# pvjosue/CWFA

Measured on AMD Instinct MI355X. Metric: volumes/sec inverse-pass @512×512×96 fp32; NLL match vs ref (1/2/4/8 GPU), higher is better.
Workload: dtype f32 (storage, accumulation, wavelets, couplings); convolution products on the bf16 matrix cores from an exact three-way bf16 split of both fp32 operands, six products per fp32 product: fp32-equivalent; plain-fp32-MFMA figure: fp32_mfma; 1 GPU; 512x512x96 volume, 4-scale CWFA (CAT blocks, 64 ch) + LRNN inverse, z=0, batch 1/GPU, random-init weights (BASELINE.json configs[2]); precision=split, parallelism=replicated x1 (independent volumes per GPU, no collective)

## Files before the change

cwfa_amd/build.py:

```python
import os
import subprocess
import sys
from concurrent.futures import ThreadPoolExecutor

HERE = os.path.dirname(os.path.abspath(__file__))
CSRC = os.path.join(HERE, "csrc")
INCLUDE = os.path.join(os.path.dirname(HERE), "include")
LIB = os.path.join(HERE, "libcwfa_hip.so")
SOURCES = ["elementwise.hip", "conv2d.hip", "conv_wino.hip", "conv_wino2d.hip", "conv_split_layer.hip", "conv_split_out.hip", "conv_split3x3.hip", "conv3d.hip", "conv3d_split.hip", "lrnn_ops.hip", "conv_bwd.hip", "eval_ops.hip", "prep_ops.hip", "optim_ops.hip", "loss_ops.hip", "deconv_ops.hip", "neuron_ops.hip", "noise_ops.hip"]
HIPCC = os.environ.get("HIPCC", "/opt/rocm/bin/hipcc")
FLAGS = ["--offload-arch=gfx950", "-O3", "-fPIC", "-std=c++17", "-ffp-contract=off", "-I", INCLUDE, "-I", CSRC,
         "-Wall", "-Wno-unused-function"]


EXTRA = {"conv3d_split.hip": ["-fno-slp-vectorize"]}


def _newer(src, dst):
    return not os.path.exists(dst) or os.path.getmtime(src) > os.path.getmtime(dst)


def build_all(force=False, verbose=False):
    deps = [os.path.join(CSRC, "common.h"), os.path.join(CSRC, "conv_internal.h"), os.path.join(CSRC, "conv_split_out_geom.h"), os.path.join(INCLUDE, "cwfa_hip.h"),
            os.path.abspath(__file__)]
    objs, jobs = [], []
    for s in SOURCES:
        src, obj = os.path.join(CSRC, s), os.path.join(CSRC, s.replace(".hip", ".o"))
        objs.append(obj)
        if force or _newer(src, obj) or any(_newer(d, obj) for d in deps):
            jobs.append([HIPCC, *FLAGS, *EXTRA.get(s, []), "-c", src, "-o", obj])

    def run(cmd):
        if verbose:
            print(" ".join(cmd), flush=True)
        r = subprocess.run(cmd, capture_output=True, text=True)
        if r.returncode != 0:
            raise RuntimeError(f"hipcc failed: {' '.join(cmd)}\n{r.stdout}\n{r.stderr}")
        return r.stderr
# ... 13 lines not shown
```

cwfa_amd/csrc/conv2d.hip:

```cpp
#include "conv_internal.h"

#include <string.h>
#include <type_traits>

namespace {

template <int KS_, int CK_, int MT_, int NT_, int WM_, int WN_, int XV_ = 1>
struct Cfg {
    static constexpr int KS = KS_, CK = CK_, MT = MT_, NT = NT_, WM = WM_, WN = WN_;
    static constexpr int XV = XV_;
    static_assert(XV_ == 1 || (XV_ == 4 && KS_ == 1), "vector staging needs halo-free tiles");
    static constexpr int PAD = KS / 2;
    static constexpr int NTHREADS = 64 * WM * WN;
    static constexpr int CT = 32 * MT * WM;
    static constexpr int TR = NT * WN;
    static constexpr int TC = 32;
    static constexpr int XR = TR + KS - 1;
    static constexpr int XC = TC + KS - 1;
    static constexpr int XS = CK * XR * XC;
    static constexpr int XS_PAD = (XS + 3) & ~3;
    static constexpr int WS = KS * KS * CK * CT;
    static constexpr int XPT = (XS / XV + NTHREADS - 1) / NTHREADS;
    static constexpr int WPT = (WS / 4 + NTHREADS - 1) / NTHREADS;
    static constexpr int BUF = XS_PAD + WS;
// ... 541 lines not shown
            return CWFA_E_SHAPE;
        default: break;
    }
    return launch_epi<C, EPI_GENERIC, PRO>(p, st);
}

template <class C, unsigned ALLOWED, unsigned ALLOWED_PRO>
int launch(const ConvParams& p, int epi, hipStream_t st) {
    if (p.o.in_scale || p.o.in_add) return launch_sel<C, ALLOWED_PRO, true>(p, epi, st);
    return launch_sel<C, ALLOWED, false>(p, epi, st);
}

}
int g_cwfa_split_xcd_map = 1;
int g_cwfa_split_rows16 = 1;
extern int g_cwfa_mip3_ablate;
namespace {

int fill_params(ConvParams& p, const char* name, const float* x, const float* w_packed, float* y, int B, int Cin, int H,
                int W, int Cout, int64_t x_bs, int64_t y_bs, const cwfa_conv_opts* opts) {
    CWFA_REQUIRE(B >= 0 && Cin > 0 && Cout > 0 && H >= 0 && W >= 0, CWFA_E_INVAL, "%s: bad size", name);
    if (B == 0 || H == 0 || W == 0) return 1;
    CWFA_REQUIRE(x && w_packed && y, CWFA_E_INVAL, "%s: null pointer", name);
    CWFA_REQUIRE(!opts || !opts->out_sample_stats, CWFA_E_INVAL, "%s: out_sample_stats is a feature of the few-channel cwfa_conv7x7_split_f32", name);
    CWFA_REQUIRE((int64_t)Cin * H * W < (1ll << 30) && (int64_t)Cout * H * W * (p.o.upshuffle2 ? 1 : 1) < (1ll << 30), CWFA_E_SHAPE, "%s: C*H*W exceeds the 32-bit byte offsets of a tile (2^30 elements per image)", name);
    CWFA_REQUIRE(cwfa_aligned16(w_packed), CWFA_E_ALIGN, "%s: packed weights must be 16-byte aligned", name);
    p.x = x; p.wp = w_packed; p.y = y;
    p.B = B; p.Cin = Cin; p.H = H; p.W = W; p.Cout = Cout;
    p.x_bs = x_bs; p.y_bs = y_bs;
    p.products = g_cwfa_operand == CwfaOperand::split3 ? 6 : 1;
// ... 308 lines not shown
    }
    if (strcmp(name, "winograd_2d") == 0) {
        g_cwfa_wino_2d = value;
        return CWFA_OK;
    }
    if (strcmp(name, "wgrad_split") == 0) {
        g_cwfa_wgrad_split = value != 0;
        return CWFA_OK;
    }
    if (strcmp(name, "wgrad_rows") == 0) {
        g_cwfa_wgrad_rows = value;
        return CWFA_OK;
    }
    if (strcmp(name, "split3x3_xcd_map") == 0) {
        g_cwfa_split_xcd_map = value;
        return CWFA_OK;
    }
    if (strcmp(name, "mip3_ablate") == 0) {
        CWFA_REQUIRE(value >= 0 && value <= 7, CWFA_E_INVAL, "cwfa_set_option: mip3_ablate is a mask of bits 0..2");
        g_cwfa_mip3_ablate = value;
        return CWFA_OK;
    }
    if (strcmp(name, "split3x3_rows16") == 0) {
        g_cwfa_split_rows16 = value;
        return CWFA_OK;
    }
    if (strcmp(name, "split_products") == 0) {
        CWFA_REQUIRE(value == 1 || value == 6, CWFA_E_INVAL, "cwfa_set_option: split_products must be 1 or 6");
        CWFA_REQUIRE(value == 1 || g_cwfa_operand != CwfaOperand::fp16, CWFA_E_INVAL,
                     "cwfa_set_option: split_products = 6 needs split_operand = 0 (the three-piece split is a bf16 format)");
// ... 130 lines not shown
```

cwfa_amd/csrc/conv_split3x3.hip:

```cpp
#include "conv_internal.h"

extern int g_cwfa_split_xcd_map;
extern int g_cwfa_split_rows16;

namespace {

constexpr int TR = 8, TC = 32;

template <int KS, int RPW = 4>
struct XG {
    static constexpr int TRW = 2 * RPW, NT = 2 * RPW;
    static constexpr int PAD = KS / 2, XR = TRW + 2 * PAD, XC = TC + 2 * PAD, NTAP = KS * KS;
    static constexpr int EPK = XR * XC;
    static constexpr int KHB = KS == 7 ? 8512 : RPW == 8 ? 9792 : 5440;
    static constexpr int XPB = 2 * KHB;
    static constexpr int XB = 3 * XPB;
    static constexpr bool SPECIAL = KS == 3 && RPW == 4;
    static constexpr int NEK = SPECIAL ? 2 : 3;
    static_assert(EPK * 16 <= KHB && KHB % 256 == 64 && 2 * EPK <= 512 * NEK, "staging entry map");
    static_assert(!SPECIAL || (EPK > 256 && EPK <= 384), "3x3 staging entry map");
    static_assert(KS == 3 || RPW == 4, "7x7: 8-row tiles");
};

template <int MPW, int KS = 3, int RPW = 4, int WM = 4>
struct Geo {
    static constexpr int CT = 16 * MPW * WM;
    static constexpr int WSL = 3 * 4 * CT * 16;
    static constexpr int LDS = 2 * XG<KS, RPW>::XB + 2 * WSL;
    static_assert(LDS <= 160 * 1024, "LDS budget");
};

struct SParams {
    const float* x;
    const void* wp;
    float* y;
    int B, Cin, H, W, Cout, nchunks, nsteps, tiles_x, ntiles, ctiles, xcd_map;
    int nrun;
    int64_t x_bs, y_bs;
    cwfa_conv_opts o;
    cwfa_couple cp;
};

template <int KS, int RPW>
__host__ __device__ constexpr int tap_off(int buf, int tap) { return buf * XG<KS, RPW>::XB + ((tap / KS) * XG<KS, RPW>::XC + tap % KS) * 16; }

enum { EPI_RUNTIME = -1, EPI_COUPLE = -2 };

template <int MPW, bool SIX, bool ADD, int ACT1, int KS = 3, int RPW = 4, int WM = 4, bool F16 = false>
__global__ __launch_bounds__(512, 1) void conv3x3_split_kernel(SParams p) {
    typedef XG<KS, RPW> G;
    constexpr int XC = G::XC, EPK = G::EPK, KHB = G::KHB, XPB = G::XPB, XB = G::XB, NTAP = G::NTAP, PAD = G::PAD;
    constexpr int WN = 8 / WM, RW = G::TRW / WN, NT = 2 * RW;
    constexpr bool SPECIAL = G::SPECIAL;
    static_assert(SPECIAL || ((MPW == 1 || WM != 4) && !ADD), "7x7 / 16-row tiles: the 64-channel and narrow tilings, without a skip add");
    static_assert(WM == 4 || (((KS == 3 && RPW == 8) || KS == 7) && MPW <= 3 && !ADD && ACT1 != EPI_COUPLE),
                  "narrow tilings: 16-row tile (7x7: 8-row), <= 3 m-tiles per wave");
    static_assert(MPW != 3 || WM != 4, "three m-tiles per wave: the 48- / 96-channel tilings only");
    constexpr int CT = 16 * MPW * WM;
    constexpr int WSL = 3 * 4 * CT * 16;
    extern __shared__ __attribute__((aligned(16))) char lds[];
    const int tid = threadIdx.x, lane = tid & 63, c16 = lane & 15, g = lane >> 4;
    const int wave = __builtin_amdgcn_readfirstlane(tid >> 6);
    const int wm = wave % WM, wn = wave / WM;
    const int HW = p.H * p.W;
    const int plane = HW * 4;
    constexpr unsigned OOB = 0x80000000u;
    constexpr int NQ = SIX ? 3 : 1;
    constexpr int OFF_W = 2 * XB;
    const int b = blockIdx.z;
    int sp, ct;
    if (p.xcd_map && (p.ntiles & 7) == 0) {
        const int xcd = blockIdx.x & 7, slot = blockIdx.x >> 3;
        sp = xcd * (p.ntiles >> 3) + slot / p.ctiles;
        ct = slot % p.ctiles;
    } else {
        sp = blockIdx.x / p.ctiles;
        ct = blockIdx.x % p.ctiles;
    }
    const int row0 = (sp / p.tiles_x) * G::TRW, col0 = (sp % p.tiles_x) * TC;

    constexpr int NEK = G::NEK;
    int ekh[NEK], eidx[NEK];
    bool fin[NEK];
    unsigned fo[NEK];
    if constexpr (SPECIAL) {
        ekh[0] = wave >> 2; eidx[0] = tid & 255; fin[0] = true;
        ekh[1] = (wave >> 1) & 1; eidx[1] = 256 + (tid & 127); fin[1] = wave < 4 && eidx[1] < EPK;
    } else {
#pragma unroll
        for (int k = 0; k < NEK; ++k) {
            const int e = tid + 512 * k;
            ekh[k] = e >= EPK;
            eidx[k] = e - ekh[k] * EPK;
            fin[k] = e < 2 * EPK;
        }
    }
    bool fok[NEK];
#pragma unroll
    for (int k = 0; k < NEK; ++k) {
        const int r = eidx[k] / XC, c = eidx[k] % XC;
        const int gr = row0 + r - PAD, gc = col0 + c - PAD;
        fok[k] = fin[k] && gr >= 0 && gr < p.H && gc >= 0 && gc < p.W;
        fo[k] = !fok[k] ? OOB : p.o.in_blocked8 ? (unsigned)((gr * p.W + gc) * 32) : (unsigned)((gr * p.W + gc) * 4);
        if constexpr (!SPECIAL) fo[k] = !fok[k] ? OOB : fo[k] + (unsigned)(ekh[k] * 8) * (unsigned)plane;
    }
    const int xbytes = p.Cin * plane;
    const auto rx = CWFA_RSRC(p.x + (int64_t)b * p.x_bs, xbytes);
    const auto ra = CWFA_RSRC(ADD ? p.o.in_add + (int64_t)b * p.o.in_add_bs : p.x, ADD ? xbytes : 0);
    const bool has_aff = p.o.in_scale != nullptr;
    typedef const float __attribute__((address_space(4))) cfloat;
    cfloat* sc = has_aff ? (cfloat*)(p.o.in_scale + (int64_t)b * p.o.in_affine_bs) : nullptr;
    cfloat* sh = has_aff ? (cfloat*)(p.o.in_shift + (int64_t)b * p.o.in_affine_bs) : nullptr;

    auto load_entry = [&](auto kc, float (&xv)[8], float (&av)[8], int chunk) {
        constexpr int k = decltype(kc)::value;
        const int ch0 = chunk * 16 + (SPECIAL ? ekh[k] * 8 : 0);
        if (KS == 3 && !ADD && p.o.in_blocked8) {
            const f32x4 lo4 = __builtin_bit_cast(f32x4, __builtin_amdgcn_raw_buffer_load_b128(rx, fo[k], ch0 * plane, 0));
            const f32x4 hi4 = __builtin_bit_cast(f32x4, __builtin_amdgcn_raw_buffer_load_b128(rx, fo[k], ch0 * plane + 16, 0));
#pragma unroll
            for (int j = 0; j < 4; ++j) {
                xv[j] = lo4[j];
                xv[4 + j] = hi4[j];
            }
            return;
        }
#pragma unroll
// ... 22 lines not shown
            float v = xv[j];
            if (has_aff) v = fok[k] ? v * scv[j] + shv[j] : 0.f;
            if constexpr (ADD) v += av[j];
            __bf16 a1, a2 = (__bf16)0.f, a3 = (__bf16)0.f;
            cwfa_split3<SIX, F16>(v, a1, a2, a3);
            pc[0][j] = a1; pc[1][j] = a2; pc[2][j] = a3;
        }
        char* dst = lds + buf * XB + ekh[k] * KHB + eidx[k] * 16;
        if (SPECIAL || fin[k]) {
#pragma unroll
            for (int q = 0; q < NQ; ++q) *reinterpret_cast<bf16x8*>(dst + q * XPB) = pc[q];
        }
    };

    constexpr int NPC = (SIX ? WSL : WSL / 3) / 1024;
    const int64_t wtile = (int64_t)ct * p.nsteps * WSL;
    const char* wbase = reinterpret_cast<const char*>(p.wp) + wtile;
    const auto rw = CWFA_RSRC(wbase, p.nsteps * WSL);
    auto dma_w = [&](int slice, int slot) {
        cwfa_static_for<(NPC + 7) / 8>([&](auto ic_) {
            constexpr int i = decltype(ic_)::value;
            const int piece = i * 8 + wave;
            if (piece < NPC) {
                char* dst = lds + OFF_W + slot * WSL + piece * 1024;
                __builtin_amdgcn_raw_ptr_buffer_load_lds(rw, (lds_ptr)dst, 16, (unsigned)(lane * 16), slice * WSL + piece * 1024, 0, 0);
            }
        });
    };

    const int alane = OFF_W + (g * CT + wm * MPW * 16 + c16) * 16;
    const int blane = (g & 1) * KHB + (wn * RW * XC + c16) * 16;
    const bool sel = (g >> 1) != 0;

    f32x4 acc[MPW][NT];
#pragma unroll
    for (int mt = 0; mt < MPW; ++mt)
#pragma unroll
        for (int nt = 0; nt < NT; ++nt) acc[mt][nt] = f32x4{0.f, 0.f, 0.f, 0.f};
    constexpr int NB = MPW == 4 ? 3 : 2, MA = MPW == 4 ? 2 : MPW;
    static_assert(NB - 1 < NT, "B look-ahead");
    bf16x8 A[MPW][3], Bq[NB][3];
    float xs[NEK][8], sk[NEK][8];

    auto read_a = [&](int abase, int m0, int m1) {
#pragma unroll
        for (int mt = m0; mt < m1; ++mt)
#pragma unroll
            for (int q = 0; q < NQ; ++q) A[mt][q] = *reinterpret_cast<const bf16x8*>(lds + abase + (q * 4 * CT + mt * 16) * 16);
    };
    auto read_b = [&](int set, int bbase, int nt) {
#pragma unroll
        for (int q = 0; q < NQ; ++q)
            Bq[set][q] = *reinterpret_cast<const bf16x8*>(lds + bbase + q * XPB + ((nt >> 1) * XC + 16 * (nt & 1)) * 16);
    };
    auto mfma6 = [&](f32x4& c, const bf16x8 (&a)[3], const bf16x8 (&bb)[3]) {
        if constexpr (SIX) {
            CWFA_MFMA(a[2], bb[0], c);
            CWFA_MFMA(a[1], bb[1], c);
            CWFA_MFMA(a[0], bb[2], c);
            CWFA_MFMA(a[1], bb[0], c);
            CWFA_MFMA(a[0], bb[1], c);
        }
        CWFA_MFMA_OP(F16, a[0], bb[0], c);
    };

    {
        float x0[NEK][8], s0[NEK][8];
        cwfa_static_for<NEK>([&](auto kc) { load_entry(kc, x0[decltype(kc)::value], s0[decltype(kc)::value], 0); });
        cwfa_static_for<NEK>([&](auto kc) { load_entry(kc, xs[decltype(kc)::value], sk[decltype(kc)::value], 1); });
        dma_w(0, 0);
        cwfa_static_for<NEK>([&](auto kc) { store_entry(kc, x0[decltype(kc)::value], s0[decltype(kc)::value], 0, 0); });
    }
    asm volatile("s_waitcnt vmcnt(0)\n\ts_waitcnt lgkmcnt(0)" ::: "memory");
    __builtin_amdgcn_s_barrier();

    read_b(0, blane + (sel ? tap_off<KS, RPW>(0, 1) : tap_off<KS, RPW>(0, 0)), 0);
    int sl = 0, P = 0, ce = 0;
    for (int step = 0; step < p.nrun; ++step) {
        const int co = ce + 1;
        const int uA = 2 * P, uB = 2 * P + 1;
        const int bufA = uA >= NTAP, tA = uA - NTAP * bufA, bufB = uB >= NTAP, tB = uB - NTAP * bufB;
        const int offA = bufA * XB + ((tA / KS) * XC + tA % KS) * 16, offB = bufB * XB + ((tB / KS) * XC + tB % KS) * 16;
        constexpr int SB = 0, SA = KS == 3 ? 5 : 26, LA = KS == 3 ? 2 : 22, LB = KS == 3 ? 6 : 44;
        static_assert(LB + NEK - 1 < NTAP && LA + NEK - 1 < SA, "staging schedule");
        static_assert(SB < LA && SA <= LB, "staging schedule: one register set per entry (a step's stores come before its loads)");
        {
            const bool odd0 = P == SB, odd1 = P == SB + 1;
            if (odd0 || P == SA) store_entry(cwfa_ic<0>{}, xs[0], sk[0], odd0 ? co : ce + 2, odd0);
            if (odd1 || P == SA + 1) store_entry(cwfa_ic<1>{}, xs[1], sk[1], odd1 ? co : ce + 2, odd1);
            if constexpr (NEK > 2) {
                const bool odd2 = P == SB + 2;
                if (odd2 || P == SA + 2) store_entry(cwfa_ic<NEK - 1>{}, xs[NEK - 1], sk[NEK - 1], odd2 ? co : ce + 2, odd2);
            }
        }
        CWFA_FENCE();
        const int abase = alane + sl * WSL;
        const int bbase = blane + (sel ? offB : offA);
        read_a(abase, 0, MA);
        CWFA_FENCE();
#pragma unroll
        for (int nt = 0; nt < NT; ++nt) {
            if ((MA == MPW || nt > 0) && nt + NB - 1 < NT) read_b((nt + NB - 1) % NB, bbase, nt + NB - 1);
            CWFA_FENCE();
#pragma unroll
            for (int mt = 0; mt < MPW; ++mt) {
                mfma6(acc[mt][nt], A[mt], Bq[nt % NB]);
                CWFA_FENCE();
                if (MA < MPW && nt == 0 && mt == 0) {
                    read_a(abase, MA, MPW);
#pragma unroll
                    for (int n2 = 1; n2 < NB && n2 < NT; ++n2) read_b(n2, bbase, n2);
                    CWFA_FENCE();
                }
            }
            if (nt == 0) {
                if (P == LA || P == LB) load_entry(cwfa_ic<0>{}, xs[0], sk[0], P == LA ? ce + 2 : co + 2);
                if (P == LA + 1 || P == LB + 1) load_entry(cwfa_ic<1>{}, xs[1], sk[1], P == LA + 1 ? ce + 2 : co + 2);
                if constexpr (NEK > 2) {
                    if (P == LA + 2 || P == LB + 2) load_entry(cwfa_ic<NEK - 1>{}, xs[NEK - 1], sk[NEK - 1], P == LA + 2 ? ce + 2 : co + 2);
                }
                CWFA_FENCE();
            }
            if (nt == 1) {
                dma_w(step + 1, sl ^ 1);
                CWFA_FENCE();
            }
        }
        {
            const int nP = P == NTAP - 1 ? 0 : P + 1;
            const int nA = 2 * nP, nB = 2 * nP + 1;
            const int nbufA = nA >= NTAP, ntA = nA - NTAP * nbufA, nbufB = nB >= NTAP, ntB = nB - NTAP * nbufB;
            const int noffA = nbufA * XB + ((ntA / KS) * XC + ntA % KS) * 16, noffB = nbufB * XB + ((ntB / KS) * XC + ntB % KS) * 16;
            read_b(0, blane + (sel ? noffB : noffA), 0);
            CWFA_FENCE();
        }
        asm volatile("s_waitcnt vmcnt(0)" ::: "memory");
        if constexpr (SIX) asm volatile("s_waitcnt lgkmcnt(3)" ::: "memory");
        else asm volatile("s_waitcnt lgkmcnt(1)" ::: "memory");
        __builtin_amdgcn_s_barrier();
        sl ^= 1;
        if (++P == NTAP) {
            P = 0;
            ce += 2;
        }
    }
    asm volatile("s_waitcnt vmcnt(0)" ::: "memory");

    const auto ry = CWFA_RSRC(p.y + (int64_t)b * p.y_bs, p.Cout * plane);
    const auto rr = CWFA_RSRC(p.o.residual ? p.o.residual + (int64_t)b * p.o.res_bs : p.y, p.o.residual ? p.Cout * plane : 0);
    const auto rb = CWFA_RSRC(p.o.bias ? p.o.bias : p.y, p.o.bias ? p.Cout * 4 : 0);
    const bool alpha_pc = p.o.prelu_per_channel != 0;
    const float alpha = (p.o.prelu_alpha && !alpha_pc) ? *p.o.prelu_alpha : 0.f;
    const auto rpa = CWFA_RSRC(alpha_pc ? p.o.prelu_alpha : p.y, alpha_pc ? p.Cout * 4 : 0);
    const int cwave = ct * CT + wm * MPW * 16;
    const unsigned glane = (unsigned)(4 * g) * (unsigned)plane;
    if constexpr (ACT1 == EPI_COUPLE) {
        static_assert(MPW <= 2 && !ADD, "coupling epilogue: narrow tilings only");
        constexpr int NP = MPW == 1 ? 2 : 4;
        const cwfa_couple& cp = p.cp;
        const auto cx = CWFA_RSRC(cp.x + (int64_t)b * cp.x_bs, cp.n * plane);
        const auto cy = CWFA_RSRC(cp.y + (int64_t)b * cp.y_bs, cp.n * plane);
        const unsigned jlane = (unsigned)((MPW == 1 ? 2 : 4) * g) * (unsigned)plane;
        const int jwave = wm * (MPW == 1 ? 8 : 16);
        float bs[NP], bt[NP];
#pragma unroll
        for (int k = 0; k < NP; ++k) {
            const int rs = k, rt = MPW == 1 ? k + 2 : 16 + k;
            bs[k] = __builtin_bit_cast(float, __builtin_amdgcn_raw_buffer_load_b32(rb, (unsigned)(16 * g), (cwave + rs) * 4, 0));
            bt[k] = __builtin_bit_cast(float, __builtin_amdgcn_raw_buffer_load_b32(rb, (unsigned)(16 * g), (cwave + rt) * 4, 0));
        }
        float ssum = 0.f;
#pragma unroll
        for (int nt = 0; nt < NT; ++nt) {
            const int row = row0 + wn * RW + (nt >> 1), col = col0 + 16 * (nt & 1) + c16;
            const bool ok = row < p.H && col < p.W;
            const unsigned po = ok ? (unsigned)((row * p.W + col) * 4) + jlane : OOB;
            float xv[NP];
#pragma unroll
            for (int k = 0; k < NP; ++k) xv[k] = __builtin_bit_cast(float, __builtin_amdgcn_raw_buffer_load_b32(cx, po, (jwave + k) * plane, 0));
#pragma unroll
            for (int k = 0; k < NP; ++k) {
                const float sr = acc[0][nt][k] + bs[k];
                float tr;
                if constexpr (MPW == 1) tr = acc[0][nt][k + 2] + bt[k];
                else tr = acc[MPW - 1][nt][k] + bt[k];
                const float sv = cwfa_soft_clamp(sr * cp.pre_scale, cp.clamp_kind, cp.clamp);
                const float tv = tr * cp.pre_scale;
                const float yv = cp.rev ? (xv[k] - tv) * __expf(-sv) : __expf(sv) * xv[k] + tv;
                __builtin_amdgcn_raw_buffer_store_b32(__builtin_bit_cast(unsigned, yv), cy, po, (jwave + k) * plane, 0);
                ssum += ok ? sv : 0.f;
            }
            CWFA_FENCE();
        }
        if (cp.logdet) {
            const double ws = cwfa_wave_sum((double)ssum);
            double* red = reinterpret_cast<double*>(lds);
            __builtin_amdgcn_s_barrier();
            if (lane == 0) red[wave] = ws;
            __syncthreads();
            if (tid == 0) {
                double tot = 0.0;
#pragma unroll
                for (int w = 0; w < 8; ++w) tot += red[w];
                atomicAdd(&cp.logdet[b], cp.rev ? -tot : tot);
            }
        }
        return;
    }
    const bool outb = p.o.out_blocked8 != 0;
    const bool want_stats = ACT1 != EPI_RUNTIME && p.o.out_stats != nullptr;
    float* red = reinterpret_cast<float*>(lds);
#pragma unroll
    for (int mt = 0; mt < MPW; ++mt) {
        float bias[4];
        float st1[4] = {0.f, 0.f, 0.f, 0.f}, st2[4] = {0.f, 0.f, 0.f, 0.f};
#pragma unroll
        for (int r = 0; r < 4; ++r)
            bias[r] = __builtin_bit_cast(float, __builtin_amdgcn_raw_buffer_load_b32(rb, (unsigned)(16 * g), (cwave + mt * 16 + r) * 4, 0));
        float al[4] = {alpha, alpha, alpha, alpha};
        if (alpha_pc) {
#pragma unroll
            for (int r = 0; r < 4; ++r)
                al[r] = __builtin_bit_cast(float, __builtin_amdgcn_raw_buffer_load_b32(rpa, (unsigned)(16 * g), (cwave + mt * 16 + r) * 4, 0));
        }
        constexpr int RLA = NT < 4 ? NT : 4;
        float rv[ACT1 == EPI_RUNTIME ? NT : 1][4];
        auto load_res = [&](int nt) {
            const int row = row0 + wn * RW + (nt >> 1), col = col0 + 16 * (nt & 1) + c16;
            const unsigned po = (row < p.H && col < p.W) ? (unsigned)((row * p.W + col) * 4) + glane : OOB;
#pragma unroll
            for (int r = 0; r < 4; ++r)
                rv[ACT1 == EPI_RUNTIME ? nt : 0][r] = __builtin_bit_cast(float, __builtin_amdgcn_raw_buffer_load_b32(rr, po, (cwave + mt * 16 + r) * plane, 0));
        };
        if constexpr (ACT1 == EPI_RUNTIME) {
#pragma unroll
            for (int nt = 0; nt < NT; ++nt)
#pragma unroll
                for (int r = 0; r < 4; ++r) rv[nt][r] = 0.f;
            if (p.o.residual) {
#pragma unroll
                for (int nt = 0; nt < RLA; ++nt) load_res(nt);
            }
            CWFA_FENCE();
        }
#pragma unroll
        for (int nt = 0; nt < NT; ++nt) {
            const int row = row0 + wn * RW + (nt >> 1), col = col0 + 16 * (nt & 1) + c16;
            if constexpr (ACT1 == EPI_RUNTIME) {
                if (nt + RLA < NT && p.o.residual) load_res(nt + RLA);
                CWFA_FENCE();
            }
            if constexpr (ACT1 != EPI_RUNTIME) {
                if (outb) {
                    f32x4 o4;
#pragma unroll
                    for (int r = 0; r < 4; ++r) o4[r] = cwfa_act_ct<ACT1>(acc[mt][nt][r] + bias[r], al[r]);
                    const unsigned pb = (row < p.H && col < p.W) ? (unsigned)(((g >> 1) * HW + row * p.W + col) * 32 + (g & 1) * 16) : OOB;
                    cwfa_buffer_store_b128(__builtin_bit_cast(u32x4, o4), ry, pb, (cwave + mt * 16) * plane);
                    continue;
                }
            }
            const unsigned po = (row < p.H && col < p.W) ? (unsigned)((row * p.W + col) * 4) + glane : OOB;
#pragma unroll
            for (int r = 0; r < 4; ++r) {
                const int soff = (cwave + mt * 16 + r) * plane;
                float v = acc[mt][nt][r] + bias[r];
                if constexpr (ACT1 == EPI_RUNTIME) {
                    v = cwfa_act(v, p.o.act, al[r]);
                    v += rv[nt][r];
                    v = cwfa_act(v, p.o.act2, al[r]);
                } else {
                    v = cwfa_act_ct<ACT1>(v, al[r]);
                    if (want_stats) {
                        const float vm = po != OOB ? v : 0.f;
                        st1[r] += vm;
                        st2[r] += vm * vm;
                    }
                }
                __builtin_amdgcn_raw_buffer_store_b32(__builtin_bit_cast(unsigned, v), ry, po, soff, 0);
            }
            CWFA_FENCE();
        }
        if constexpr (ACT1 != EPI_RUNTIME) {
            if (want_stats) {
#pragma unroll
                for (int r = 0; r < 4; ++r) {
                    const float a1 = cwfa_row16_sum(st1[r]), a2 = cwfa_row16_sum(st2[r]);
                    if (c16 == 0) {
                        const int ch = (wm * MPW + mt) * 16 + 4 * g + r;
                        red[(wn * CT + ch) * 2] = a1;
                        red[(wn * CT + ch) * 2 + 1] = a2;
                    }
                }
            }
        }
    }
    if constexpr (ACT1 != EPI_RUNTIME) {
        if (want_stats) {
            asm volatile("s_waitcnt lgkmcnt(0)\n\ts_barrier" ::: "memory");
            const int ch = ct * CT + tid;
            if (tid < CT && ch < p.Cout) {
                double s1 = 0.0, s2 = 0.0;
#pragma unroll
                for (int k = 0; k < WN; ++k) {
                    s1 += (double)red[(k * CT + tid) * 2];
                    s2 += (double)red[(k * CT + tid) * 2 + 1];
                }
                atomicAdd(&p.o.out_stats[2 * ch], s1);
                atomicAdd(&p.o.out_stats[2 * ch + 1], s2);
            }
        }
    }
}

namespace few {
constexpr int XR = TR + 6, XC = TC + 6, EPK = XR * XC;
constexpr int XPB = EPK * 16;
constexpr int NSTEP = 13, CT = 64, MPW = 2, WM = 2, WN = 4, RW = 2, NT = 4;
constexpr int WSL = 3 * 4 * CT * 16;
constexpr int OFF_W = 3 * XPB, LDS = OFF_W + 2 * WSL;
static_assert(2 * 512 >= EPK && 2 * LDS <= 160 * 1024, "few-channel 7x7: staging map / two blocks per CU");
}

template <bool SIX, bool F16>
__global__ __launch_bounds__(512, 2) void conv7x7_few_split_kernel(SParams p) {
    using namespace few;
// ... 234 lines not shown
    for (int q = 0; q < 3; ++q) {
        uint4 v4;
        v4.x = pc[q][0] | ((unsigned)pc[q][1] << 16);
        v4.y = pc[q][2] | ((unsigned)pc[q][3] << 16);
        v4.z = pc[q][4] | ((unsigned)pc[q][5] << 16);
        v4.w = pc[q][6] | ((unsigned)pc[q][7] << 16);
        out[(((int64_t)ctile * nsteps + s) * 3 + q) * 4 * CT + g * CT + col] = v4;
    }
}

inline int mpw_of(int Cout) { return Cout > 128 ? 4 : Cout > 96 ? 2 : Cout > 64 ? 3 : Cout > 48 ? 1 : Cout > 32 ? 3 : Cout > 16 ? 2 : 1; }
inline int wm_of(int Cout) { return Cout > 96 ? 4 : Cout > 64 ? 2 : Cout > 48 ? 4 : 1; }
inline int ct_of(int Cout) { return 16 * mpw_of(Cout) * wm_of(Cout); }
inline int nsteps_of(int Cin, int ntap = 9) { return ntap * (((Cin + 15) / 16 + 1) / 2); }

template <int MPW, bool ADD, int ACT1, int KS = 3, int RPW = 4, int WM = 4>
int launch(const SParams& p, hipStream_t stream) {
    typedef Geo<MPW, KS, RPW, WM> G;
    constexpr int TRW = XG<KS, RPW>::TRW;
    const int tiles_y = (p.H + TRW - 1) / TRW, ctiles = (p.Cout + G::CT - 1) / G::CT;
    SParams q = p;
    q.ntiles = p.tiles_x * tiles_y;
    q.ctiles = ctiles;
    q.xcd_map = g_cwfa_split_xcd_map;
    if ((int64_t)q.ntiles * ctiles >= (1ll << 31)) {
        cwfa_set_error("cwfa_conv3x3_split_f32: grid too large");
        return CWFA_E_SHAPE;
    }
    if ((ACT1 == EPI_RUNTIME || ACT1 == EPI_COUPLE) && (p.o.out_stats || p.o.out_blocked8)) {
        cwfa_set_error("cwfa_conv3x3_split_f32: out_stats / out_blocked8 reached a run-time epilogue");
        return CWFA_E_INVAL;
    }
    return cwfa_with_operand([&](auto six, auto f16) -> int {
        constexpr auto kern = &conv3x3_split_kernel<MPW, six, ADD, ACT1, KS, RPW, WM, f16>;
        const int rc = cwfa_max_lds<kern>(G::LDS, "cwfa_conv3x3_split_f32");
        if (rc) return rc;
        hipLaunchKernelGGL(kern, dim3((unsigned)(q.ntiles * ctiles), 1, p.B), dim3(512), G::LDS, stream, q);
        CWFA_LAUNCH_CHECK("cwfa_conv3x3_split_f32");
        return CWFA_OK;
    });
}

template <int MPW>
int launch_epi(const SParams& p, hipStream_t st) {
    const bool plain = !p.o.residual && p.o.act2 == CWFA_ACT_NONE;
    if (p.o.in_add) {
        if (plain && p.o.act == CWFA_ACT_PRELU) return launch<MPW, true, CWFA_ACT_PRELU>(p, st);
        return launch<MPW, true, EPI_RUNTIME>(p, st);
    }
    if (plain && p.o.act == CWFA_ACT_PRELU) return launch<MPW, false, CWFA_ACT_PRELU>(p, st);
    if (plain && p.o.act == CWFA_ACT_NONE) return launch<MPW, false, CWFA_ACT_NONE>(p, st);
    return launch<MPW, false, EPI_RUNTIME>(p, st);
// ... 221 lines not shown
```

cwfa_amd/ops.py:

```python
import ctypes as C

import torch

from . import _lib
from ._lib import AffineStage, Chain, ConvOpts, check

__all__ = ["haar1d", "haar2d", "gather", "affine", "channel_affine", "chain_inv", "chain_inv_var", "chain_inv_roi_cov", "chain_inv_samples", "rand_uniform", "rand_trunc_normal", "rand_poisson", "chain_nll_map", "nll_compose", "chain_fwd", "pack_conv_weight",
           "conv2d", "conv2d_wgrad", "elu_bwd", "set_precision", "gelu_add", "gelu_bwd", "layernorm_bwd", "attention_bwd", "plane_affine", "bn_bwd_stats", "bn_act_bwd", "maxpool2_bwd", "chain_bwd", "chain_inv_bwd", "prelu_bwd", "conv3d_1k1_backward", "pack_1x1_panel", "pack_split_layer_weight", "subnet_layer", "conv3d_1k1", "channel_stats", "bn_fold", "bn_running_update", "maxpool", "sample_stats", "layernorm_apply",
           "convnext_tail", "conv_writes_sample_stats", "attention_combine", "scale_channels", "axpby", "stage", "lion_step", "global_extrema", "wmse_loss"]


def _stream():
    return C.c_void_p(torch.cuda.current_stream().cuda_stream)


def _p(t):
    return None if t is None else C.c_void_p(t.data_ptr())


def _dev(t, name="tensor"):
    if not torch.is_tensor(t):
        raise TypeError(f"{name}: expected a torch.Tensor, got {type(t)}")
    if not t.is_cuda:
        raise RuntimeError(f"{name}: cwfa_amd runs on MI355X only -- got a {t.device} tensor (no CPU fallback exists)")
# ... 714 lines not shown
    elif pc.split and pc.ks == 3:
        if split3x3_narrow(pc.cout) and (in_scale is not None or in_add is not None):
            if (H * W) % 4 == 0:
                x = plane_affine(x, in_scale, in_shift, add=in_add)
            else:
                if in_scale is not None:
                    if in_scale.numel() == Cin:
                        x = channel_affine(x, in_scale.reshape(-1), in_shift.reshape(-1))
                    else:
                        x = torch.cat([channel_affine(x[i:i + 1], in_scale.reshape(B, Cin)[i].contiguous(), in_shift.reshape(B, Cin)[i].contiguous())
                                       for i in range(B)], 0)
                if in_add is not None:
                    x = axpby(x.contiguous(), 1.0, in_add, 1.0)
            x, xbs = planes(x, "x")
            o.in_scale = o.in_shift = o.in_add = None
        check(L.cwfa_conv3x3_split_f32(_p(x), _p(pc.packed), _p(out), B, Cin, H, W, pc.cout, xbs, ybs, C.byref(o),
                                       _stream()), "conv3x3_split")
    elif pc.split:
        ws = torch.empty(L.cwfa_split_workspace_bytes(B, Cin, H * W), dtype=torch.uint8, device=x.device)
        per_sample = in_scale is not None and in_scale.numel() == B * Cin and B > 1
        check(L.cwfa_split_input_f32(_p(x), _p(ws), B, Cin, H * W, xbs, _p(in_scale), _p(in_shift), Cin if per_sample else 0,
                                     _p(in_add), in_add.stride(0) if in_add is not None else 0, _stream()), "split_input")
        o.in_scale = o.in_shift = o.in_add = None
        check(L.cwfa_conv_split_f32(_p(ws), _p(pc.packed), _p(out), B, Cin, H, W, pc.cout, pc.ks, ybs, C.byref(o), _stream()),
              "conv_split")
    else:
        check(L.cwfa_conv2d_f32(_p(x), _p(pc.packed), _p(out), B, Cin, H, W, pc.cout, pc.ks, xbs, ybs, C.byref(o),
                                _stream()), "conv2d")
    if rec is not None and rec.want(key):
        e1.record()
# ... 37 lines not shown
    o2, obs = planes(out, "out")
    if tuple(x.shape) != (B, n, H, W) or tuple(out.shape) != (B, n, H, W) or o2.data_ptr() != out.data_ptr():
        raise ValueError("conv3x3_couple: x / out must be [B,n,H,W] views with contiguous planes")
    cp = _lib.Couple()
    cp.x, cp.y, cp.x_bs, cp.y_bs, cp.n = x2.data_ptr(), out.data_ptr(), xbs, obs, n
    cp.clamp_kind, cp.clamp, cp.pre_scale, cp.rev = _lib.CLAMP[clamp_kind], float(clamp), float(pre_scale), int(bool(rev))
    if logdet is not None:
        cp.logdet = logdet.data_ptr()
    cp.in_blocked8 = int(bool(in_blocked))
    rec = conv_event_sink
    if rec is not None:
        key = (3, Cin, pc.cout, H, W, B, "||||couple+split", False)
        if rec.want(key):
            e0, e1 = torch.cuda.Event(enable_timing=True), torch.cuda.Event(enable_timing=True)
            e0.record()
    check(L.cwfa_conv3x3_split_couple_f32(_p(u), _p(pc.packed), _p(br), B, Cin, H, W, ubs, C.byref(cp), _stream()),
          "conv3x3_split_couple")
    if rec is not None and rec.want(key):
        e1.record()
        rec.add(key, e0, e1)
    return out


BLOCKED_MAPS = True
SPLIT_7X7 = True
VIRTUAL_CAT = True
COUPLE_EPILOGUE = True


def couple_fused():
    return COUPLE_EPILOGUE and _split_bf16 >= 2


def split3x3_narrow(cout):
    return cout <= 48 or 64 < cout <= 96

# ... 657 lines not shown


def pack_epoch():
    return _pack_epoch


def invalidate_packs():
    global _pack_epoch
    _pack_epoch += 1


WINOGRAD_2D_DEFAULT = 512


def set_option(name, value):
    global _split_bf16, _pack_epoch
    _pack_epoch += 1
    if name == "split_bf16":
        _split_bf16 = int(value)
        return
    check(_lib.lib().cwfa_set_option(name.encode(), int(value)), "set_option")


PRECISIONS = ("fp32", "split_bf16", "bf16", "fp16")


def set_precision(mode):
    if mode not in PRECISIONS:
        raise ValueError(f"set_precision: unknown mode {mode!r}")
    global _precision
    _precision = mode
# ... 668 lines not shown
```

Before: 57.72 volumes/s.

## Make split 3x3 conv kernel persistent with cross-tile prefetch of next tile

Turns the 3x3 split-bf16 conv kernel into a persistent kernel: the grid is capped at the CU count, and each workgroup walks several (batch, spatial, channel) tiles. While the current tile finishes, it stages the next tile's input halo and first weight slice. The epilogue uses a free weight ring slot as scratch instead of the input LDS area, so the epilogue can overlap with prefetched data. This targets launch tail and the per-tile pipeline fill and drain cost. In exchange it adds register pressure, more kernarg reloads and extra complexity in the schedule.

New measurement: 58.01 volumes/s, median of 6. No clear change (+0.5%).

```diff
diff --git a/cwfa_amd/build.py b/cwfa_amd/build.py
--- a/cwfa_amd/build.py
+++ b/cwfa_amd/build.py
@@ -21,7 +21,8 @@
 
 
 def build_all(force=False, verbose=False):
-    deps = [os.path.join(CSRC, "common.h"), os.path.join(CSRC, "conv_internal.h"), os.path.join(CSRC, "conv_split_out_geom.h"), os.path.join(INCLUDE, "cwfa_hip.h"),
+    deps = [os.path.join(CSRC, "common.h"), os.path.join(CSRC, "conv_internal.h"), os.path.join(CSRC, "conv_split_out_geom.h"), os.path.join(CSRC, "conv_split3x3_walk.h"),
+            os.path.join(INCLUDE, "cwfa_hip.h"),
             os.path.abspath(__file__)]
     objs, jobs = [], []
     for s in SOURCES:
diff --git a/cwfa_amd/csrc/conv2d.hip b/cwfa_amd/csrc/conv2d.hip
--- a/cwfa_amd/csrc/conv2d.hip
+++ b/cwfa_amd/csrc/conv2d.hip
@@ -579,6 +579,8 @@
 }
 int g_cwfa_split_xcd_map = 1;
 int g_cwfa_split_rows16 = 1;
+int g_cwfa_split_persistent = 1;
+int g_cwfa_split_max_wg = 0;
 extern int g_cwfa_mip3_ablate;
 namespace {
 
@@ -917,6 +919,15 @@
     }
     if (strcmp(name, "split3x3_xcd_map") == 0) {
         g_cwfa_split_xcd_map = value;
+        return CWFA_OK;
+    }
+    if (strcmp(name, "split3x3_persistent") == 0) {
+        g_cwfa_split_persistent = value != 0;
+        return CWFA_OK;
+    }
+    if (strcmp(name, "split3x3_max_workgroups") == 0) {
+        CWFA_REQUIRE(value >= 0, CWFA_E_INVAL, "cwfa_set_option: split3x3_max_workgroups must be >= 0");
+        g_cwfa_split_max_wg = value;
         return CWFA_OK;
     }
     if (strcmp(name, "mip3_ablate") == 0) {
diff --git a/cwfa_amd/csrc/conv_split3x3.hip b/cwfa_amd/csrc/conv_split3x3.hip
--- a/cwfa_amd/csrc/conv_split3x3.hip
+++ b/cwfa_amd/csrc/conv_split3x3.hip
@@ -1,6 +1,9 @@
 #include "conv_internal.h"
+#include "conv_split3x3_walk.h"
 
 extern int g_cwfa_split_xcd_map;
+extern int g_cwfa_split_persistent;
+extern int g_cwfa_split_max_wg;
 extern int g_cwfa_split_rows16;
 
 namespace {
@@ -35,6 +38,7 @@
     const void* wp;
     float* y;
     int B, Cin, H, W, Cout, nchunks, nsteps, tiles_x, ntiles, ctiles, xcd_map;
+    int total;
     int nrun;
     int64_t x_bs, y_bs;
     cwfa_conv_opts o;
@@ -45,6 +49,9 @@
 __host__ __device__ constexpr int tap_off(int buf, int tap) { return buf * XG<KS, RPW>::XB + ((tap / KS) * XG<KS, RPW>::XC + tap % KS) * 16; }
 
 enum { EPI_RUNTIME = -1, EPI_COUPLE = -2 };
+
+template <int MPW, bool SIX, bool ADD, int KS>
+constexpr bool walk_form() { return KS == 3 && !(MPW == 4 && SIX && ADD); }
 
 template <int MPW, bool SIX, bool ADD, int ACT1, int KS = 3, int RPW = 4, int WM = 4, bool F16 = false>
 __global__ __launch_bounds__(512, 1) void conv3x3_split_kernel(SParams p) {
@@ -67,17 +74,22 @@
     constexpr unsigned OOB = 0x80000000u;
     constexpr int NQ = SIX ? 3 : 1;
     constexpr int OFF_W = 2 * XB;
-    const int b = blockIdx.z;
-    int sp, ct;
-    if (p.xcd_map && (p.ntiles & 7) == 0) {
-        const int xcd = blockIdx.x & 7, slot = blockIdx.x >> 3;
-        sp = xcd * (p.ntiles >> 3) + slot / p.ctiles;
-        ct = slot % p.ctiles;
-    } else {
-        sp = blockIdx.x / p.ctiles;
-        ct = blockIdx.x % p.ctiles;
-    }
-    const int row0 = (sp / p.tiles_x) * G::TRW, col0 = (sp % p.tiles_x) * TC;
+    const bool xmap = cwfa_walk3::xcd_walk(p.xcd_map, p.ntiles, (int64_t)gridDim.x);
+    typedef const SParams __attribute__((address_space(4))) CSParams;
+    auto args = [&]() -> CSParams& {
+        CSParams* qp = (CSParams*)__builtin_amdgcn_kernarg_segment_ptr();
+        asm volatile("" : "+s"(qp));
+        return *qp;
+    };
+    int sb, srow0, scol0, sct;
+    auto stage_coords = [&](int it) {
+        CSParams& q = args();
+        int sp;
+        cwfa_walk3::tile_of(it, xmap, q.ntiles, q.ctiles, sb, sp, sct);
+        const int ty = sp / q.tiles_x;
+        srow0 = ty * G::TRW;
+        scol0 = (sp - ty * q.tiles_x) * TC;
+    };
 
     constexpr int NEK = G::NEK;
     int ekh[NEK], eidx[NEK];
@@ -96,21 +108,28 @@
         }
     }
     bool fok[NEK];
-#pragma unroll
-    for (int k = 0; k < NEK; ++k) {
-        const int r = eidx[k] / XC, c = eidx[k] % XC;
-        const int gr = row0 + r - PAD, gc = col0 + c - PAD;
-        fok[k] = fin[k] && gr >= 0 && gr < p.H && gc >= 0 && gc < p.W;
-        fo[k] = !fok[k] ? OOB : p.o.in_blocked8 ? (unsigned)((gr * p.W + gc) * 32) : (unsigned)((gr * p.W + gc) * 4);
-        if constexpr (!SPECIAL) fo[k] = !fok[k] ? OOB : fo[k] + (unsigned)(ekh[k] * 8) * (unsigned)plane;
-    }
     const int xbytes = p.Cin * plane;
-    const auto rx = CWFA_RSRC(p.x + (int64_t)b * p.x_bs, xbytes);
-    const auto ra = CWFA_RSRC(ADD ? p.o.in_add + (int64_t)b * p.o.in_add_bs : p.x, ADD ? xbytes : 0);
     const bool has_aff = p.o.in_scale != nullptr;
     typedef const float __attribute__((address_space(4))) cfloat;
-    cfloat* sc = has_aff ? (cfloat*)(p.o.in_scale + (int64_t)b * p.o.in_affine_bs) : nullptr;
-    cfloat* sh = has_aff ? (cfloat*)(p.o.in_shift + (int64_t)b * p.o.in_affine_bs) : nullptr;
+    cfloat *sc = nullptr, *sh = nullptr;
+    auto rx = CWFA_RSRC(p.x, 0), ra = CWFA_RSRC(p.x, 0);
+    auto stage_map = [&]() {
+        CSParams& q = args();
+#pragma unroll
+        for (int k = 0; k < NEK; ++k) {
+            int e = eidx[k];
+            asm volatile("" : "+v"(e));
+            const int r = e / XC, c = e % XC;
+            const int gr = srow0 + r - PAD, gc = scol0 + c - PAD;
+            fok[k] = fin[k] && gr >= 0 && gr < q.H && gc >= 0 && gc < q.W;
+            fo[k] = !fok[k] ? OOB : q.o.in_blocked8 ? (unsigned)((gr * q.W + gc) * 32) : (unsigned)((gr * q.W + gc) * 4);
+            if constexpr (!SPECIAL) fo[k] = !fok[k] ? OOB : fo[k] + (unsigned)(ekh[k] * 8) * (unsigned)plane;
+        }
+        rx = CWFA_RSRC(q.x + (int64_t)sb * q.x_bs, xbytes);
+        ra = CWFA_RSRC(ADD ? q.o.in_add + (int64_t)sb * q.o.in_add_bs : q.x, ADD ? xbytes : 0);
+        sc = has_aff ? (cfloat*)(q.o.in_scale + (int64_t)sb * q.o.in_affine_bs) : nullptr;
+        sh = has_aff ? (cfloat*)(q.o.in_shift + (int64_t)sb * q.o.in_affine_bs) : nullptr;
+    };
 
     auto load_entry = [&](auto kc, float (&xv)[8], float (&av)[8], int chunk) {
         constexpr int k = decltype(kc)::value;
@@ -163,9 +182,11 @@
     };
 
     constexpr int NPC = (SIX ? WSL : WSL / 3) / 1024;
-    const int64_t wtile = (int64_t)ct * p.nsteps * WSL;
-    const char* wbase = reinterpret_cast<const char*>(p.wp) + wtile;
-    const auto rw = CWFA_RSRC(wbase, p.nsteps * WSL);
+    auto rw = CWFA_RSRC(p.wp, 0);
+    auto weights_of = [&](int ct) {
+        CSParams& q = args();
+        rw = CWFA_RSRC(reinterpret_cast<const char*>(q.wp) + (int64_t)ct * q.nsteps * WSL, q.nsteps * WSL);
+    };
     auto dma_w = [&](int slice, int slot) {
         cwfa_static_for<(NPC + 7) / 8>([&](auto ic_) {
             constexpr int i = decltype(ic_)::value;
@@ -182,10 +203,6 @@
     const bool sel = (g >> 1) != 0;
 
     f32x4 acc[MPW][NT];
-#pragma unroll
-    for (int mt = 0; mt < MPW; ++mt)
-#pragma unroll
-        for (int nt = 0; nt < NT; ++nt) acc[mt][nt] = f32x4{0.f, 0.f, 0.f, 0.f};
     constexpr int NB = MPW == 4 ? 3 : 2, MA = MPW == 4 ? 2 : MPW;
     static_assert(NB - 1 < NT, "B look-ahead");
     bf16x8 A[MPW][3], Bq[NB][3];
@@ -213,6 +230,10 @@
         CWFA_MFMA_OP(F16, a[0], bb[0], c);
     };
 
+    int it = blockIdx.x;
+    stage_coords(it);
+    stage_map();
+    weights_of(sct);
     {
         float x0[NEK][8], s0[NEK][8];
         cwfa_static_for<NEK>([&](auto kc) { load_entry(kc, x0[decltype(kc)::value], s0[decltype(kc)::value], 0); });
@@ -223,10 +244,23 @@
     asm volatile("s_waitcnt vmcnt(0)\n\ts_waitcnt lgkmcnt(0)" ::: "memory");
     __builtin_amdgcn_s_barrier();
 
+    const int nchp = 2 * (p.nsteps / NTAP);
+    const bool trimmed = p.nrun != p.nsteps;
+    int sl = 0;
+    for (;;) {
+    const int b = sb, row0 = srow0, col0 = scol0, ct = sct;
+    const unsigned itn = (unsigned)it + gridDim.x;
+    const bool has_next = walk_form<MPW, SIX, ADD, KS>() && itn < (unsigned)p.total;
+#pragma unroll
+    for (int mt = 0; mt < MPW; ++mt)
+#pragma unroll
+        for (int nt = 0; nt < NT; ++nt) acc[mt][nt] = f32x4{0.f, 0.f, 0.f, 0.f};
     read_b(0, blane + (sel ? tap_off<KS, RPW>(0, 1) : tap_off<KS, RPW>(0, 0)), 0);
-    int sl = 0, P = 0, ce = 0;
+    int P = 0, ce = 0;
     for (int step = 0; step < p.nrun; ++step) {
+        const bool lastp = ce + 2 >= nchp, stage_on = !lastp || has_next;
         const int co = ce + 1;
+        const int nce = lastp ? 0 : ce + 2, nco = nce + 1;
         const int uA = 2 * P, uB = 2 * P + 1;
         const int bufA = uA >= NTAP, tA = uA - NTAP * bufA, bufB = uB >= NTAP, tB = uB - NTAP * bufB;
         const int offA = bufA * XB + ((tA / KS) * XC + tA % KS) * 16, offB = bufB * XB + ((tB / KS) * XC + tB % KS) * 16;
@@ -235,11 +269,11 @@
         static_assert(SB < LA && SA <= LB, "staging schedule: one register set per entry (a step's stores come before its loads)");
         {
             const bool odd0 = P == SB, odd1 = P == SB + 1;
-            if (odd0 || P == SA) store_entry(cwfa_ic<0>{}, xs[0], sk[0], odd0 ? co : ce + 2, odd0);
-            if (odd1 || P == SA + 1) store_entry(cwfa_ic<1>{}, xs[1], sk[1], odd1 ? co : ce + 2, odd1);
+            if (odd0 || (P == SA && stage_on)) store_entry(cwfa_ic<0>{}, xs[0], sk[0], odd0 ? co : nce, odd0);
+            if (odd1 || (P == SA + 1 && stage_on)) store_entry(cwfa_ic<1>{}, xs[1], sk[1], odd1 ? co : nce, odd1);
             if constexpr (NEK > 2) {
                 const bool odd2 = P == SB + 2;
-                if (odd2 || P == SA + 2) store_entry(cwfa_ic<NEK - 1>{}, xs[NEK - 1], sk[NEK - 1], odd2 ? co : ce + 2, odd2);
+                if (odd2 || (P == SA + 2 && stage_on)) store_entry(cwfa_ic<NEK - 1>{}, xs[NEK - 1], sk[NEK - 1], odd2 ? co : nce, odd2);
             }
         }
         CWFA_FENCE();
@@ -263,15 +297,24 @@
                 }
             }
             if (nt == 0) {
-                if (P == LA || P == LB) load_entry(cwfa_ic<0>{}, xs[0], sk[0], P == LA ? ce + 2 : co + 2);
-                if (P == LA + 1 || P == LB + 1) load_entry(cwfa_ic<1>{}, xs[1], sk[1], P == LA + 1 ? ce + 2 : co + 2);
+                if (P == LA && lastp && has_next) {
+                    stage_coords((int)itn);
+                    stage_map();
+                }
+                if ((P == LA || P == LB) && stage_on) load_entry(cwfa_ic<0>{}, xs[0], sk[0], P == LA ? nce : nco);
+                if ((P == LA + 1 || P == LB + 1) && stage_on) load_entry(cwfa_ic<1>{}, xs[1], sk[1], P == LA + 1 ? nce : nco);
                 if constexpr (NEK > 2) {
-                    if (P == LA + 2 || P == LB + 2) load_entry(cwfa_ic<NEK - 1>{}, xs[NEK - 1], sk[NEK - 1], P == LA + 2 ? ce + 2 : co + 2);
+                    if ((P == LA + 2 || P == LB + 2) && stage_on) load_entry(cwfa_ic<NEK - 1>{}, xs[NEK - 1], sk[NEK - 1], P == LA + 2 ? nce : nco);
                 }
                 CWFA_FENCE();
             }
             if (nt == 1) {
-                dma_w(step + 1, sl ^ 1);
+                if (step + 1 < p.nrun) {
+                    dma_w(step + 1, sl ^ 1);
+                } else if (has_next) {
+                    weights_of(sct);
+                    dma_w(0, sl ^ 1);
+                }
                 CWFA_FENCE();
             }
         }
@@ -293,20 +336,34 @@
             ce += 2;
         }
     }
-    asm volatile("s_waitcnt vmcnt(0)" ::: "memory");
-
-    const auto ry = CWFA_RSRC(p.y + (int64_t)b * p.y_bs, p.Cout * plane);
-    const auto rr = CWFA_RSRC(p.o.residual ? p.o.residual + (int64_t)b * p.o.res_bs : p.y, p.o.residual ? p.Cout * plane : 0);
-    const auto rb = CWFA_RSRC(p.o.bias ? p.o.bias : p.y, p.o.bias ? p.Cout * 4 : 0);
-    const bool alpha_pc = p.o.prelu_per_channel != 0;
-    const float alpha = (p.o.prelu_alpha && !alpha_pc) ? *p.o.prelu_alpha : 0.f;
-    const auto rpa = CWFA_RSRC(alpha_pc ? p.o.prelu_alpha : p.y, alpha_pc ? p.Cout * 4 : 0);
+    if (trimmed && has_next) {
+        cwfa_static_for<NEK>([&](auto kc) { store_entry(kc, xs[decltype(kc)::value], sk[decltype(kc)::value], 0, 0); });
+        CWFA_FENCE();
+        cwfa_static_for<NEK>([&](auto kc) { load_entry(kc, xs[decltype(kc)::value], sk[decltype(kc)::value], 1); });
+        CWFA_FENCE();
+    }
+    char* const scratch = lds + OFF_W + (sl ^ 1) * WSL;
+    bool endbar = trimmed;
+    static_assert(8 * 16 * MPW * 8 <= WSL, "epilogue scratch fits a ring slot");
+
+    {
+    CSParams& q = args();
+    int tid_e = threadIdx.x;
+    asm volatile("" : "+v"(tid_e));
+    const int tid = tid_e, lane = tid & 63, c16 = lane & 15, g = lane >> 4;
+    const int HW = q.H * q.W, plane = HW * 4;
+    const auto ry = CWFA_RSRC(q.y + (int64_t)b * q.y_bs, q.Cout * plane);
+    const auto rr = CWFA_RSRC(q.o.residual ? q.o.residual + (int64_t)b * q.o.res_bs : q.y, q.o.residual ? q.Cout * plane : 0);
+    const auto rb = CWFA_RSRC(q.o.bias ? q.o.bias : q.y, q.o.bias ? q.Cout * 4 : 0);
+    const bool alpha_pc = q.o.prelu_per_channel != 0;
+    const float alpha = (q.o.prelu_alpha && !alpha_pc) ? *q.o.prelu_alpha : 0.f;
+    const auto rpa = CWFA_RSRC(alpha_pc ? q.o.prelu_alpha : q.y, alpha_pc ? q.Cout * 4 : 0);
     const int cwave = ct * CT + wm * MPW * 16;
     const unsigned glane = (unsigned)(4 * g) * (unsigned)plane;
     if constexpr (ACT1 == EPI_COUPLE) {
         static_assert(MPW <= 2 && !ADD, "coupling epilogue: narrow tilings only");
         constexpr int NP = MPW == 1 ? 2 : 4;
-        const cwfa_couple& cp = p.cp;
+        const auto& cp = q.cp;
         const auto cx = CWFA_RSRC(cp.x + (int64_t)b * cp.x_bs, cp.n * plane);
         const auto cy = CWFA_RSRC(cp.y + (int64_t)b * cp.y_bs, cp.n * plane);
         const unsigned jlane = (unsigned)((MPW == 1 ? 2 : 4) * g) * (unsigned)plane;
@@ -322,8 +379,8 @@
 #pragma unroll
         for (int nt = 0; nt < NT; ++nt) {
             const int row = row0 + wn * RW + (nt >> 1), col = col0 + 16 * (nt & 1) + c16;
-            const bool ok = row < p.H && col < p.W;
-            const unsigned po = ok ? (unsigned)((row * p.W + col) * 4) + jlane : OOB;
+            const bool ok = row < q.H && col < q.W;
+            const unsigned po = ok ? (unsigned)((row * q.W + col) * 4) + jlane : OOB;
             float xv[NP];
 #pragma unroll
             for (int k = 0; k < NP; ++k) xv[k] = __builtin_bit_cast(float, __builtin_amdgcn_raw_buffer_load_b32(cx, po, (jwave + k) * plane, 0));
@@ -343,7 +400,7 @@
         }
         if (cp.logdet) {
             const double ws = cwfa_wave_sum((double)ssum);
-            double* red = reinterpret_cast<double*>(lds);
+            double* red = reinterpret_cast<double*>(scratch);
             __builtin_amdgcn_s_barrier();
             if (lane == 0) red[wave] = ws;
             __syncthreads();
@@ -353,12 +410,12 @@
                 for (int w = 0; w < 8; ++w) tot += red[w];
                 atomicAdd(&cp.logdet[b], cp.rev ? -tot : tot);
             }
-        }
-        return;
-    }
-    const bool outb = p.o.out_blocked8 != 0;
-    const bool want_stats = ACT1 != EPI_RUNTIME && p.o.out_stats != nullptr;
-    float* red = reinterpret_cast<float*>(lds);
+            endbar = true;
+        }
+    } else {
+    const bool outb = q.o.out_blocked8 != 0;
+    const bool want_stats = ACT1 != EPI_RUNTIME && q.o.out_stats != nullptr;
+    float* red = reinterpret_cast<float*>(scratch);
 #pragma unroll
     for (int mt = 0; mt < MPW; ++mt) {
         float bias[4];
@@ -376,7 +433,7 @@
         float rv[ACT1 == EPI_RUNTIME ? NT : 1][4];
         auto load_res = [&](int nt) {
             const int row = row0 + wn * RW + (nt >> 1), col = col0 + 16 * (nt & 1) + c16;
-            const unsigned po = (row < p.H && col < p.W) ? (unsigned)((row * p.W + col) * 4) + glane : OOB;
+            const unsigned po = (row < q.H && col < q.W) ? (unsigned)((row * q.W + col) * 4) + glane : OOB;
 #pragma unroll
             for (int r = 0; r < 4; ++r)
                 rv[ACT1 == EPI_RUNTIME ? nt : 0][r] = __builtin_bit_cast(float, __builtin_amdgcn_raw_buffer_load_b32(rr, po, (cwave + mt * 16 + r) * plane, 0));
@@ -386,7 +443,7 @@
             for (int nt = 0; nt < NT; ++nt)
 #pragma unroll
                 for (int r = 0; r < 4; ++r) rv[nt][r] = 0.f;
-            if (p.o.residual) {
+            if (q.o.residual) {
 #pragma unroll
                 for (int nt = 0; nt < RLA; ++nt) load_res(nt);
             }
@@ -396,7 +453,7 @@
         for (int nt = 0; nt < NT; ++nt) {
             const int row = row0 + wn * RW + (nt >> 1), col = col0 + 16 * (nt & 1) + c16;
             if constexpr (ACT1 == EPI_RUNTIME) {
-                if (nt + RLA < NT && p.o.residual) load_res(nt + RLA);
+                if (nt + RLA < NT && q.o.residual) load_res(nt + RLA);
                 CWFA_FENCE();
             }
             if constexpr (ACT1 != EPI_RUNTIME) {
@@ -404,20 +461,20 @@
                     f32x4 o4;
 #pragma unroll
                     for (int r = 0; r < 4; ++r) o4[r] = cwfa_act_ct<ACT1>(acc[mt][nt][r] + bias[r], al[r]);
-                    const unsigned pb = (row < p.H && col < p.W) ? (unsigned)(((g >> 1) * HW + row * p.W + col) * 32 + (g & 1) * 16) : OOB;
+                    const unsigned pb = (row < q.H && col < q.W) ? (unsigned)(((g >> 1) * HW + row * q.W + col) * 32 + (g & 1) * 16) : OOB;
                     cwfa_buffer_store_b128(__builtin_bit_cast(u32x4, o4), ry, pb, (cwave + mt * 16) * plane);
                     continue;
                 }
             }
-            const unsigned po = (row < p.H && col < p.W) ? (unsigned)((row * p.W + col) * 4) + glane : OOB;
+            const unsigned po = (row < q.H && col < q.W) ? (unsigned)((row * q.W + col) * 4) + glane : OOB;
 #pragma unroll
             for (int r = 0; r < 4; ++r) {
                 const int soff = (cwave + mt * 16 + r) * plane;
                 float v = acc[mt][nt][r] + bias[r];
                 if constexpr (ACT1 == EPI_RUNTIME) {
-                    v = cwfa_act(v, p.o.act, al[r]);
+                    v = cwfa_act(v, q.o.act, al[r]);
                     v += rv[nt][r];
-                    v = cwfa_act(v, p.o.act2, al[r]);
+                    v = cwfa_act(v, q.o.act2, al[r]);
                 } else {
                     v = cwfa_act_ct<ACT1>(v, al[r]);
                     if (want_stats) {
@@ -448,17 +505,24 @@
         if (want_stats) {
             asm volatile("s_waitcnt lgkmcnt(0)\n\ts_barrier" ::: "memory");
             const int ch = ct * CT + tid;
-            if (tid < CT && ch < p.Cout) {
+            if (tid < CT && ch < q.Cout) {
                 double s1 = 0.0, s2 = 0.0;
 #pragma unroll
                 for (int k = 0; k < WN; ++k) {
                     s1 += (double)red[(k * CT + tid) * 2];
                     s2 += (double)red[(k * CT + tid) * 2 + 1];
                 }
-                atomicAdd(&p.o.out_stats[2 * ch], s1);
-                atomicAdd(&p.o.out_stats[2 * ch + 1], s2);
-            }
-        }
+                atomicAdd(&q.o.out_stats[2 * ch], s1);
+                atomicAdd(&q.o.out_stats[2 * ch + 1], s2);
+            }
+            endbar = true;
+        }
+    }
+    }
+    }
+    if (!has_next) break;
+    if (endbar) asm volatile("s_waitcnt lgkmcnt(0)\n\ts_barrier" ::: "memory");
+    it = (int)itn;
     }
 }
 
@@ -723,6 +787,8 @@
 inline int ct_of(int Cout) { return 16 * mpw_of(Cout) * wm_of(Cout); }
 inline int nsteps_of(int Cin, int ntap = 9) { return ntap * (((Cin + 15) / 16 + 1) / 2); }
 
+int g_num_cus = 0;
+
 template <int MPW, bool ADD, int ACT1, int KS = 3, int RPW = 4, int WM = 4>
 int launch(const SParams& p, hipStream_t stream) {
     typedef Geo<MPW, KS, RPW, WM> G;
@@ -732,9 +798,19 @@
     q.ntiles = p.tiles_x * tiles_y;
     q.ctiles = ctiles;
     q.xcd_map = g_cwfa_split_xcd_map;
-    if ((int64_t)q.ntiles * ctiles >= (1ll << 31)) {
+    const int64_t total = cwfa_walk3::total_tiles(q.ntiles, ctiles, p.B);
+    if (total >= (1ll << 31)) {
         cwfa_set_error("cwfa_conv3x3_split_f32: grid too large");
         return CWFA_E_SHAPE;
+    }
+    q.total = (int)total;
+    if (g_cwfa_split_persistent && g_cwfa_split_max_wg <= 0 && g_num_cus == 0) {
+        int dev = 0, n = 0;
+        if (hipGetDevice(&dev) != hipSuccess || hipDeviceGetAttribute(&n, hipDeviceAttributeMultiprocessorCount, dev) != hipSuccess || n <= 0) {
+            cwfa_set_error("cwfa_conv3x3_split_f32: cannot query the CU count");
+            return CWFA_E_HIP;
+        }
+        g_num_cus = n;
     }
     if ((ACT1 == EPI_RUNTIME || ACT1 == EPI_COUPLE) && (p.o.out_stats || p.o.out_blocked8)) {
         cwfa_set_error("cwfa_conv3x3_split_f32: out_stats / out_blocked8 reached a run-time epilogue");
@@ -744,7 +820,9 @@
         constexpr auto kern = &conv3x3_split_kernel<MPW, six, ADD, ACT1, KS, RPW, WM, f16>;
         const int rc = cwfa_max_lds<kern>(G::LDS, "cwfa_conv3x3_split_f32");
         if (rc) return rc;
-        hipLaunchKernelGGL(kern, dim3((unsigned)(q.ntiles * ctiles), 1, p.B), dim3(512), G::LDS, stream, q);
+        const bool walk = g_cwfa_split_persistent && walk_form<MPW, six, ADD, KS>();
+        const unsigned grid = (unsigned)cwfa_walk3::grid_of(total, g_num_cus, walk, g_cwfa_split_max_wg);
+        hipLaunchKernelGGL(kern, dim3(grid), dim3(512), G::LDS, stream, q);
         CWFA_LAUNCH_CHECK("cwfa_conv3x3_split_f32");
         return CWFA_OK;
     });
diff --git a/cwfa_amd/csrc/conv_split3x3_walk.h b/cwfa_amd/csrc/conv_split3x3_walk.h
--- /dev/null
+++ b/cwfa_amd/csrc/conv_split3x3_walk.h
@@ -0,0 +1,38 @@
+#pragma once
+#include <cstdint>
+
+#if defined(__HIPCC__) || defined(__CUDACC__)
+#define CWFA_WALK3_HD __host__ __device__
+#else
+#define CWFA_WALK3_HD
+#endif
+
+namespace cwfa_walk3 {
+
+CWFA_WALK3_HD constexpr int64_t total_tiles(int ntiles, int ctiles, int B) { return (int64_t)ntiles * ctiles * B; }
+
+CWFA_WALK3_HD constexpr int64_t grid_of(int64_t total, int cus, int persistent, int cap) {
+    if (!persistent) return total;
+    const int64_t lim = cap > 0 ? cap : cus;
+    return total < lim ? total : lim;
+}
+
+CWFA_WALK3_HD constexpr bool xcd_walk(int xcd_map, int ntiles, int64_t grid) { return xcd_map && (ntiles & 7) == 0 && (grid & 7) == 0; }
+
+CWFA_WALK3_HD constexpr void tile_of(int it, bool xmap, int ntiles, int ctiles, int& b, int& sp, int& ct) {
+    if (xmap) {
+        const int band = ntiles >> 3, per = band * ctiles, slot = it >> 3;
+        b = slot / per;
+        const int rem = slot - b * per, s = rem / ctiles;
+        sp = (it & 7) * band + s;
+        ct = rem - s * ctiles;
+    } else {
+        const int per = ntiles * ctiles;
+        b = it / per;
+        const int rem = it - b * per;
+        sp = rem / ctiles;
+        ct = rem - sp * ctiles;
+    }
+}
+
+}
diff --git a/cwfa_amd/ops.py b/cwfa_amd/ops.py
--- a/cwfa_amd/ops.py
+++ b/cwfa_amd/ops.py
@@ -752,6 +752,7 @@
                     x = axpby(x.contiguous(), 1.0, in_add, 1.0)
             x, xbs = planes(x, "x")
             o.in_scale = o.in_shift = o.in_add = None
+        _sync_split3x3_walk()
         check(L.cwfa_conv3x3_split_f32(_p(x), _p(pc.packed), _p(out), B, Cin, H, W, pc.cout, xbs, ybs, C.byref(o),
                                        _stream()), "conv3x3_split")
     elif pc.split:
@@ -819,12 +820,24 @@
         if rec.want(key):
             e0, e1 = torch.cuda.Event(enable_timing=True), torch.cuda.Event(enable_timing=True)
             e0.record()
+    _sync_split3x3_walk()
     check(L.cwfa_conv3x3_split_couple_f32(_p(u), _p(pc.packed), _p(br), B, Cin, H, W, ubs, C.byref(cp), _stream()),
           "conv3x3_split_couple")
     if rec is not None and rec.want(key):
         e1.record()
         rec.add(key, e0, e1)
     return out
+
+
+SPLIT3X3_WALK = True
+_split3x3_walk_set = True
+
+
+def _sync_split3x3_walk():
+    global _split3x3_walk_set
+    if bool(SPLIT3X3_WALK) != _split3x3_walk_set:
+        check(_lib.lib().cwfa_set_option(b"split3x3_persistent", int(bool(SPLIT3X3_WALK))), "set_option")
+        _split3x3_walk_set = bool(SPLIT3X3_WALK)
 
 
 BLOCKED_MAPS = True
@@ -1512,7 +1525,12 @@
 
 
 def set_option(name, value):
-    global _split_bf16, _pack_epoch
+    global _split_bf16, _pack_epoch, SPLIT3X3_WALK, _split3x3_walk_set
+    if name in ("split3x3_persistent", "split3x3_max_workgroups"):
+        check(_lib.lib().cwfa_set_option(name.encode(), int(value)), "set_option")
+        if name == "split3x3_persistent":
+            SPLIT3X3_WALK = _split3x3_walk_set = bool(value)
+        return
     _pack_epoch += 1
     if name == "split_bf16":
         _split_bf16 = int(value)
```
